# babbu3682/MTD-GAN

Hardware: AMD Instinct MI355X
Metric: GAN train-step imgs/sec (G+D fwd+bwd) @ 64x64 patch (higher is better)
Workload: dtype f32; 1 GPU; Full G+D+PCGrad train step (BASELINE configs[2]; configs[3] when N>1); per_gpu_batch=32, global_batch=32, patch=1x64x64, parallelism=dp1

## Files before the change

mtd-gan_amd/csrc/fft64.h:

```cpp
#pragma once
#include "common.h"

namespace {

__device__ __constant__ const float COS64[32] = {
    1.f, 0.995184727f, 0.98078528f, 0.956940336f, 0.923879533f, 0.881921264f, 0.831469612f, 0.773010453f,
    0.707106781f, 0.634393284f, 0.555570233f, 0.471396737f, 0.382683432f, 0.290284677f, 0.195090322f, 0.0980171403f,
    0.f, -0.0980171403f, -0.195090322f, -0.290284677f, -0.382683432f, -0.471396737f, -0.555570233f, -0.634393284f,
    -0.707106781f, -0.773010453f, -0.831469612f, -0.881921264f, -0.923879533f, -0.956940336f, -0.98078528f, -0.995184727f};
__device__ __constant__ const float SIN64[32] = {
    0.f, 0.0980171403f, 0.195090322f, 0.290284677f, 0.382683432f, 0.471396737f, 0.555570233f, 0.634393284f,
    0.707106781f, 0.773010453f, 0.831469612f, 0.881921264f, 0.923879533f, 0.956940336f, 0.98078528f, 0.995184727f,
    1.f, 0.995184727f, 0.98078528f, 0.956940336f, 0.923879533f, 0.881921264f, 0.831469612f, 0.773010453f,
    0.707106781f, 0.634393284f, 0.555570233f, 0.471396737f, 0.382683432f, 0.290284677f, 0.195090322f, 0.0980171403f};

__host__ __device__ constexpr int brev6(int k) {
    return ((k & 1) << 5) | ((k & 2) << 3) | ((k & 4) << 1) | ((k & 8) >> 1) | ((k & 16) >> 3) | ((k & 32) >> 5);
}

template <int SIGN>
__device__ __forceinline__ void fft64(float (&re)[64], float (&im)[64]) {
#pragma unroll
    for (int s = 0; s < 6; ++s) {
        const int half = 32 >> s;
        const int tstep = 1 << s;
#pragma unroll
        for (int blk = 0; blk < 64; blk += 2 * half) {
#pragma unroll
            for (int j = 0; j < half; ++j) {
                const int i0 = blk + j, i1 = i0 + half;
                const float ar = re[i0], ai = im[i0], br = re[i1], bi = im[i1];
                re[i0] = ar + br;
                im[i0] = ai + bi;
                const float dr = ar - br, di = ai - bi;
                const int tw = j * tstep;
                if (tw == 0) {
                    re[i1] = dr;
                    im[i1] = di;
                } else if (tw == 16) {
                    if (SIGN < 0) { re[i1] = di; im[i1] = -dr; }
                    else { re[i1] = -di; im[i1] = dr; }
                } else {
                    const float c = COS64[tw];
                    const float sn = (SIGN < 0) ? -SIN64[tw] : SIN64[tw];
                    re[i1] = dr * c - di * sn;
                    im[i1] = dr * sn + di * c;
                }
            }
        }
    }
}

__host__ __device__ constexpr int brev4(int k) { return ((k & 1) << 3) | ((k & 2) << 1) | ((k & 4) >> 1) | ((k & 8) >> 3); }

template <int SIGN>
__device__ __forceinline__ void fft16(float (&re)[16], float (&im)[16]) {
#pragma unroll
    for (int s = 0; s < 4; ++s) {
        const int half = 8 >> s;
        const int tstep = 1 << s;
#pragma unroll
        for (int blk = 0; blk < 16; blk += 2 * half) {
#pragma unroll
            for (int j = 0; j < half; ++j) {
                const int i0 = blk + j, i1 = i0 + half;
                const float ar = re[i0], ai = im[i0], br = re[i1], bi = im[i1];
                re[i0] = ar + br;
                im[i0] = ai + bi;
                const float dr = ar - br, di = ai - bi;
                const int tw = j * tstep;
                if (tw == 0) {
                    re[i1] = dr;
                    im[i1] = di;
                } else if (tw == 4) {
                    if (SIGN < 0) { re[i1] = di; im[i1] = -dr; }
                    else { re[i1] = -di; im[i1] = dr; }
                } else {
                    const float c = COS64[4 * tw];
                    const float sn = (SIGN < 0) ? -SIN64[4 * tw] : SIN64[4 * tw];
                    re[i1] = dr * c - di * sn;
                    im[i1] = dr * sn + di * c;
                }
            }
        }
    }
}

__device__ __forceinline__ float quad_bcast(float v, int k) {
    const int x = __builtin_bit_cast(int, v);
    int r;
    switch (k) {
        case 0: r = __builtin_amdgcn_update_dpp(0, x, 0x00, 0xf, 0xf, true); break;
        case 1: r = __builtin_amdgcn_update_dpp(0, x, 0x55, 0xf, 0xf, true); break;
        case 2: r = __builtin_amdgcn_update_dpp(0, x, 0xAA, 0xf, 0xf, true); break;
        default: r = __builtin_amdgcn_update_dpp(0, x, 0xFF, 0xf, 0xf, true); break;
    }
    return __builtin_bit_cast(float, r);
}

template <int SIGN>
__device__ __forceinline__ void fft64_quad(float (&re)[16], float (&im)[16], const float (&tc)[16], const float (&ts)[16], int j) {
    fft16<SIGN>(re, im);
    float gr[16], gi[16];
#pragma unroll
    for (int r = 0; r < 16; ++r) {
        const float fr = re[brev4(r)], fi = im[brev4(r)];
        if (SIGN < 0) { gr[r] = fr * tc[r] + fi * ts[r]; gi[r] = fi * tc[r] - fr * ts[r]; }
        else { gr[r] = fr * tc[r] - fi * ts[r]; gi[r] = fi * tc[r] + fr * ts[r]; }
    }
    const bool odd = (j & 1) != 0;
    const float sgn = (j & 2) ? -1.f : 1.f;
#pragma unroll
    for (int r = 0; r < 16; ++r) {
        const float g0r = quad_bcast(gr[r], 0), g1r = quad_bcast(gr[r], 1), g2r = quad_bcast(gr[r], 2), g3r = quad_bcast(gr[r], 3);
        const float g0i = quad_bcast(gi[r], 0), g1i = quad_bcast(gi[r], 1), g2i = quad_bcast(gi[r], 2), g3i = quad_bcast(gi[r], 3);
        const float ar = g0r + g2r, ai = g0i + g2i, br = g0r - g2r, bi = g0i - g2i;
        const float cr = g1r + g3r, ci = g1i + g3i, dr = g1r - g3r, di = g1i - g3i;
        const float base_r = odd ? br : ar, base_i = odd ? bi : ai;
        const float add_r = odd ? (SIGN < 0 ? di : -di) : cr;
        const float add_i = odd ? (SIGN < 0 ? -dr : dr) : ci;
        re[r] = fmaf(sgn, add_r, base_r);
        im[r] = fmaf(sgn, add_i, base_i);
    }
}

__device__ __forceinline__ void quad_twiddles(int j, float (&tc)[16], float (&ts)[16]) {
#pragma unroll
    for (int r = 0; r < 16; ++r) {
        const int idx = j * r;
        const float s = (idx & 32) ? -1.f : 1.f;
        tc[r] = s * COS64[idx & 31];
        ts[r] = s * SIN64[idx & 31];
    }
}

__device__ __forceinline__ void quad_twiddles_sel(int j, float (&tc)[16], float (&ts)[16]) {
#pragma unroll
    for (int r = 0; r < 16; ++r) {
        const float c1 = COS64[r], s1 = SIN64[r];
        const float c2 = ((2 * r) & 32) ? -COS64[(2 * r) & 31] : COS64[(2 * r) & 31];
        const float s2 = ((2 * r) & 32) ? -SIN64[(2 * r) & 31] : SIN64[(2 * r) & 31];
        const float c3 = ((3 * r) & 32) ? -COS64[(3 * r) & 31] : COS64[(3 * r) & 31];
        const float s3 = ((3 * r) & 32) ? -SIN64[(3 * r) & 31] : SIN64[(3 * r) & 31];
        tc[r] = j == 0 ? 1.f : (j == 1 ? c1 : (j == 2 ? c2 : c3));
        ts[r] = j == 0 ? 0.f : (j == 1 ? s1 : (j == 2 ? s2 : s3));
    }
}

constexpr int NKW = 33;

__device__ __forceinline__ void rfft_rows_body(const float* __restrict__ x, int x_ld, float* __restrict__ R, int npairs, int col_weight,
                                               int pair, int c) {
    if (pair >= npairs) return;
    const int b = pair >> 5, h = (pair & 31) * 2;
    float re[64], im[64];
    const float* r0 = x + ((long long)(b * 64 + h) * 64) * x_ld + c;
    const float* r1 = r0 + (long long)64 * x_ld;
#pragma unroll
    for (int w = 0; w < 64; ++w) {
        re[w] = r0[(long long)w * x_ld];
        im[w] = r1[(long long)w * x_ld];
    }
    fft64<-1>(re, im);
    float* o0 = R + ((long long)(b * NKW) * 64 + h) * 64 + c;
#pragma unroll
    for (int kw = 0; kw <= 32; ++kw) {
        const int km = (64 - kw) & 63;
        const float zkr = re[brev6(kw)], zki = im[brev6(kw)];
        const float zmr = re[brev6(km)], zmi = im[brev6(km)];
        float sc = 0.125f * 0.5f;
        if (col_weight && kw != 0 && kw != 32) sc *= 2.f;
        const float ar = (zkr + zmr) * sc, ai = (zki - zmi) * sc;
        const float br = (zki + zmi) * sc, bi = (zmr - zkr) * sc;
        float* o = o0 + (long long)kw * 64 * 64;
        o[0] = ar;
        o[32] = ai;
        o[64] = br;
        o[64 + 32] = bi;
    }
}

}
```

mtd-gan_amd/csrc/resfft4.hip:

```cpp
#include "common.h"
#include "fft64.h"

namespace {

constexpr int XLD4 = 65;
constexpr int MIX_SLAB4 = 64 * 64 + 128;
typedef __attribute__((address_space(3))) float lds_float4k;

__device__ __forceinline__ void dma_columns(const float* gsrc, float* lds_dst, int wave, int lane, bool two) {
    const int n = two ? 32 : 16;
    for (int i = wave; i < n; i += 4)
        __builtin_amdgcn_global_load_lds(gsrc + i * 256 + lane * 4, (lds_float4k*)(lds_dst + i * 256), 16, 0, 0);
}

__device__ __forceinline__ void store_rows32(const float* lds_rows, int ld, float* gdst, int lane) {
#pragma unroll
    for (int it = 0; it < 8; ++it) {
        const int row = it * 4 + (lane >> 4), q = lane & 15;
        const float* s = lds_rows + row * ld + 4 * q;
        const f32x4 v = {s[0], s[1], s[2], s[3]};
        *reinterpret_cast<f32x4*>(gdst + row * 64 + 4 * q) = v;
    }
}

__device__ __forceinline__ void stagger_wait(int lin, int d, int m) {
    if (d > 0) {
        const int n = ((lin >> 8) % m) * d;
        for (int i = 0; i < n; ++i) __builtin_amdgcn_s_sleep(16);
    }
}

__device__ __forceinline__ int mask_word(int k2, int kh, int o) {
    const int i = kh >> 5, r32 = kh & 31;
    const int e = (r32 & 3) + 4 * (r32 >> 3);
    return ((k2 * 2 + i) * 2 + (o >> 5)) * 16 + e;
}
__device__ __forceinline__ int mask_bit(int kh, int o) { return (o & 31) + 32 * (((kh & 31) >> 2) & 1); }

template <int COLS>
__global__ __launch_bounds__(128 * COLS, 3) void spec_mix_fwd4_kernel(const float* __restrict__ R, const float* __restrict__ w2t,
                                                               const float* __restrict__ b2, float* __restrict__ T,
                                                               float* __restrict__ S_save, unsigned long long* __restrict__ zmask,
                                                               int stg_d, int stg_m) {
    __shared__ __attribute__((aligned(1024))) float Xs[COLS * 64 * XLD4];
    float* const Xin = Xs;
    const int tid = threadIdx.x, lane = tid & 63;
    const int wave = __builtin_amdgcn_readfirstlane(tid >> 6);
    const int b = blockIdx.y;
    const int kw0 = COLS == 2 ? 2 * (int)blockIdx.x : (int)blockIdx.x;
    const int unit = b * 17 + (kw0 >> 1);
    const int kpos = COLS == 2 ? 0 : (kw0 & 1);
    const bool two = COLS == 2 && (kw0 + 1) < NKW;
    const long long cb0 = ((long long)(b * NKW + kw0) * 64) * 64;
    {
        const int n = two ? 32 : 16;
        for (int i = wave; i < n; i += 2 * COLS)
            __builtin_amdgcn_global_load_lds(R + cb0 + i * 256 + lane * 4, (lds_float4k*)(Xin + i * 256), 16, 0, 0);
    }
    stagger_wait(blockIdx.y * gridDim.x + blockIdx.x, stg_d, stg_m);
    const int f = tid >> 2, j = tid & 3, kwl = f >> 5, c = f & 31;
    const bool valid = kwl == 0 || two;
    float tc[16], ts[16];
    quad_twiddles(j, tc, ts);
    const int l31 = lane & 31, kh2 = lane >> 5;
    const int k2 = wave >> 1, ih = wave & 1;
    const bool mix_valid = k2 == 0 || two;
    asm volatile("s_waitcnt vmcnt(0)" ::: "memory");
    __syncthreads();
    float re[16], im[16];
    {
        const float* src = Xin + kwl * 4096 + j * 64 + c;
#pragma unroll
        for (int m = 0; m < 16; ++m) {
            re[m] = valid ? src[m * 256] : 0.f;
            im[m] = valid ? src[m * 256 + 32] : 0.f;
        }
        __syncthreads();
        fft64_quad<-1>(re, im, tc, ts, j);
#pragma unroll
        for (int r = 0; r < 16; ++r) {
            const int kh = 16 * j + r;
            const float sr = re[r] * 0.125f, si = im[r] * 0.125f;
            Xs[(kwl * 64 + kh) * XLD4 + c] = sr;
            Xs[(kwl * 64 + kh) * XLD4 + 32 + c] = si;
        }
    }
    float wf0[32], wf1[32];
#pragma unroll
    for (int kk = 0; kk < 32; ++kk) {
        wf0[kk] = w2t[(2 * kk + kh2) * 64 + l31];
        wf1[kk] = w2t[(2 * kk + kh2) * 64 + 32 + l31];
    }
    __syncthreads();
    if (mix_valid) {
        if (S_save) store_rows32(Xs + (k2 * 64 + ih * 32) * XLD4, XLD4, S_save + cb0 + (k2 * 64 + ih * 32) * 64, lane);
        f32x16 acc[2];
#pragma unroll
        for (int jj = 0; jj < 2; ++jj)
#pragma unroll
            for (int e = 0; e < 16; ++e) acc[jj][e] = 0.f;
        const float* arow = Xs + (k2 * 64 + ih * 32 + l31) * XLD4 + kh2;
#pragma unroll
        for (int kk = 0; kk < 32; ++kk) {
            const float a0 = arow[2 * kk];
            acc[0] = mfma32(a0, wf0[kk], acc[0]);
            acc[1] = mfma32(a0, wf1[kk], acc[1]);
        }
        __builtin_amdgcn_wave_barrier();
#pragma unroll
        for (int jj = 0; jj < 2; ++jj) {
            const int o = jj * 32 + l31;
            const float bo = b2[o];
#pragma unroll
            for (int e = 0; e < 16; ++e) {
                const int kh = ih * 32 + mfma32_row(e, lane);
                const float z = acc[jj][e] + bo;
                if (zmask) {
                    const unsigned long long bm = __ballot(z > 0.f);
                    if (lane == 0) zmask[(long long)unit * 128 + (((k2 + kpos) * 2 + ih) * 2 + jj) * 16 + e] = bm;
                }
                Xs[(k2 * 64 + kh) * XLD4 + o] = z > 0.f ? z : 0.f;
            }
        }
    }
    __syncthreads();
    {
        const float* src = Xs + (kwl * 64 + j) * XLD4 + c;
#pragma unroll
        for (int m = 0; m < 16; ++m) {
            re[m] = src[4 * m * XLD4];
            im[m] = src[4 * m * XLD4 + 32];
        }
        __syncthreads();
        fft64_quad<+1>(re, im, tc, ts, j);
        float* st = Xin + kwl * 4096 + c;
#pragma unroll
        for (int r = 0; r < 16; ++r) {
            const int h = 16 * j + r;
            st[h * 64] = re[r] * 0.125f;
            st[h * 64 + 32] = im[r] * 0.125f;
        }
    }
    __syncthreads();
    if (mix_valid) store_rows32(Xin + (k2 * 64 + ih * 32) * 64, 64, T + cb0 + (k2 * 64 + ih * 32) * 64, lane);
}

__global__ __launch_bounds__(256, 3) void spec_mix_bwd4_kernel(const float* __restrict__ gR, const float* __restrict__ w2,
                                                               const float* __restrict__ S_save,
                                                               const unsigned long long* __restrict__ zmask, float* __restrict__ gT,
                                                               float* __restrict__ ws, int stg_d, int stg_m) {
    __shared__ __attribute__((aligned(1024))) float Gs[2 * 64 * XLD4];
    __shared__ unsigned long long Zm[128];
    float* const Xin = Gs;
    const int tid = threadIdx.x, lane = tid & 63;
    const int wave = __builtin_amdgcn_readfirstlane(tid >> 6);
    const int b = blockIdx.y, unit = b * gridDim.x + blockIdx.x;
    const bool two = (2 * blockIdx.x + 1) < NKW;
    const long long cb0 = ((long long)(b * NKW + 2 * blockIdx.x) * 64) * 64;
    float* slab = ws + (long long)unit * MIX_SLAB4;
    dma_columns(gR + cb0, Xin, wave, lane, two);
    if (tid < 128) Zm[tid] = zmask[(long long)unit * 128 + tid];
    stagger_wait(unit, stg_d, stg_m);
    const int f = tid >> 2, j = tid & 3, kwl = f >> 5, c = f & 31;
    const bool valid = kwl == 0 || two;
    const int l31 = lane & 31, kh2 = lane >> 5;
    asm volatile("s_waitcnt vmcnt(0)" ::: "memory");
    __syncthreads();
    float re[16], im[16];
    const int io = wave >> 1, jk = wave & 1;
    float sf[32];
    {
        const float* sp = S_save + cb0 + kh2 * 64 + jk * 32 + l31;
#pragma unroll
        for (int kk = 0; kk < 32; ++kk) sf[kk] = sp[2 * kk * 64];
    }
    __builtin_amdgcn_sched_barrier(0);
    {
        float tc[16], ts[16];
        quad_twiddles(j, tc, ts);
        const float* src = Xin + kwl * 4096 + j * 64 + c;
#pragma unroll
        for (int m = 0; m < 16; ++m) {
            re[m] = valid ? src[m * 256] : 0.f;
            im[m] = valid ? src[m * 256 + 32] : 0.f;
        }
        __syncthreads();
        fft64_quad<-1>(re, im, tc, ts, j);
        float dbr = 0.f, dbi = 0.f;
#pragma unroll
        for (int r = 0; r < 16; ++r) {
            const int kh = 16 * j + r;
            float gr = re[r] * 0.125f, gi = im[r] * 0.125f;
            const unsigned long long mr = Zm[mask_word(kwl, kh, c)], mi = Zm[mask_word(kwl, kh, 32 + c)];
            const int bit = mask_bit(kh, c);
            gr = (valid && ((mr >> bit) & 1ull)) ? gr : 0.f;
            gi = (valid && ((mi >> bit) & 1ull)) ? gi : 0.f;
            dbr += gr;
            dbi += gi;
            Gs[(kwl * 64 + kh) * XLD4 + c] = gr;
            Gs[(kwl * 64 + kh) * XLD4 + 32 + c] = gi;
        }
        const float sr = ((quad_bcast(dbr, 0) + quad_bcast(dbr, 1)) + quad_bcast(dbr, 2)) + quad_bcast(dbr, 3);
        const float si = ((quad_bcast(dbi, 0) + quad_bcast(dbi, 1)) + quad_bcast(dbi, 2)) + quad_bcast(dbi, 3);
        if (j == 0) {
            slab[64 * 64 + kwl * 64 + c] = sr;
            slab[64 * 64 + kwl * 64 + 32 + c] = si;
        }
    }
    const int k2 = wave >> 1, ih = wave & 1;
    const bool mix_valid = k2 == 0 || two;
    f32x16 accd[2];
#pragma unroll
    for (int jj = 0; jj < 2; ++jj)
#pragma unroll
        for (int e = 0; e < 16; ++e) accd[jj][e] = 0.f;
    {
        float wf0[32], wf1[32];
#pragma unroll
        for (int kk = 0; kk < 32; ++kk) {
            wf0[kk] = w2[(2 * kk + kh2) * 64 + l31];
            wf1[kk] = w2[(2 * kk + kh2) * 64 + 32 + l31];
        }
        __syncthreads();
        if (mix_valid) {
            const float* arow = Gs + (k2 * 64 + ih * 32 + l31) * XLD4 + kh2;
#pragma unroll
            for (int kk = 0; kk < 32; ++kk) {
                const float a0 = arow[2 * kk];
                accd[0] = mfma32(a0, wf0[kk], accd[0]);
                accd[1] = mfma32(a0, wf1[kk], accd[1]);
            }
        }
    }
    {
        f32x16 accw;
#pragma unroll
        for (int e = 0; e < 16; ++e) accw[e] = 0.f;
        float sg[32];
        if (two) {
            const float* sp = S_save + cb0 + 4096 + kh2 * 64 + jk * 32 + l31;
#pragma unroll
            for (int kk = 0; kk < 32; ++kk) sg[kk] = sp[2 * kk * 64];
        }
        {
            const float* ga = Gs + kh2 * XLD4 + io * 32 + l31;
#pragma unroll
            for (int kk = 0; kk < 32; ++kk) accw = mfma32(ga[2 * kk * XLD4], sf[kk], accw);
        }
        if (two) {
            const float* ga = Gs + (64 + kh2) * XLD4 + io * 32 + l31;
#pragma unroll
            for (int kk = 0; kk < 32; ++kk) accw = mfma32(ga[2 * kk * XLD4], sg[kk], accw);
        }
#pragma unroll
        for (int e = 0; e < 16; ++e) slab[(io * 32 + mfma32_row(e, lane)) * 64 + jk * 32 + l31] = accw[e];
    }
    __syncthreads();
    if (mix_valid) {
#pragma unroll
        for (int jj = 0; jj < 2; ++jj)
#pragma unroll
            for (int e = 0; e < 16; ++e) Gs[(k2 * 64 + ih * 32 + mfma32_row(e, lane)) * XLD4 + jj * 32 + l31] = accd[jj][e];
    }
    __syncthreads();
    {
        float tc[16], ts[16];
        quad_twiddles(j, tc, ts);
        const float* src = Gs + (kwl * 64 + j) * XLD4 + c;
#pragma unroll
        for (int m = 0; m < 16; ++m) {
            re[m] = src[4 * m * XLD4];
            im[m] = src[4 * m * XLD4 + 32];
        }
        __syncthreads();
        fft64_quad<+1>(re, im, tc, ts, j);
        const int kw = 2 * blockIdx.x + kwl;
        const float sc = (kw == 0 || kw == 32) ? 0.125f : 0.0625f;
        float* st = Xin + kwl * 4096 + c;
#pragma unroll
        for (int r = 0; r < 16; ++r) {
            const int h = 16 * j + r;
            st[h * 64] = re[r] * sc;
            st[h * 64 + 32] = im[r] * sc;
        }
    }
    __syncthreads();
    if (mix_valid) store_rows32(Xin + (k2 * 64 + ih * 32) * 64, 64, gT + cb0 + (k2 * 64 + ih * 32) * 64, lane);
}

}

extern "C" size_t mtd_spec_mix_zmask_bytes(int B) { return B > 0 ? (size_t)B * 17 * 128 * sizeof(unsigned long long) : 0; }

extern "C" int mtd_spec_mix_fwd4(const float* R, const float* w2t, const float* b2, float* T, float* S_save, void* zmask, int B,
                                 void* stream) {
    if (!R || !w2t || !b2 || !T || B <= 0) return MTD_EINVAL;
    if (!aligned16(R)) return MTD_EALIGN;
    static const int env_cols = [] { const char* e = mtd_lab_env("MTD_SPECMIX_COLS"); return e ? atoi(e) : 1; }();
    static const int stg_d = [] { const char* e = mtd_lab_env("MTD_SPECMIX_STAGGER"); return e ? atoi(e) : 0; }();
    static const int stg_m = [] { const char* e = mtd_lab_env("MTD_SPECMIX_STAGGER_MOD"); return e ? atoi(e) : 2; }();
    if (env_cols == 2)
        hipLaunchKernelGGL((spec_mix_fwd4_kernel<2>), dim3(17, B), dim3(256), 0, (hipStream_t)stream, R, w2t, b2, T, S_save,
                           (unsigned long long*)zmask, stg_d, stg_m);
    else
        hipLaunchKernelGGL((spec_mix_fwd4_kernel<1>), dim3(NKW, B), dim3(128), 0, (hipStream_t)stream, R, w2t, b2, T, S_save,
                           (unsigned long long*)zmask, stg_d, stg_m);
    MTD_LAUNCH_CHECK();
    return MTD_OK;
}

extern "C" int mtd_spec_mix_bwd4(const float* gR, const float* w2, const float* S_save, const void* zmask, float* gT, float* ws, int B,
                                 void* stream) {
    if (!gR || !w2 || !S_save || !zmask || !gT || !ws || B <= 0) return MTD_EINVAL;
    if (!aligned16(gR) || !aligned16(S_save)) return MTD_EALIGN;
    static const int stg_d = [] { const char* e = mtd_lab_env("MTD_SPECMIX_STAGGER_BWD"); return e ? atoi(e) : 0; }();
    static const int stg_m = [] { const char* e = mtd_lab_env("MTD_SPECMIX_STAGGER_MOD"); return e ? atoi(e) : 2; }();
    hipLaunchKernelGGL(spec_mix_bwd4_kernel, dim3(17, B), dim3(256), 0, (hipStream_t)stream, gR, w2, S_save,
                       (const unsigned long long*)zmask, gT, ws, stg_d, stg_m);
    MTD_LAUNCH_CHECK();
    return MTD_OK;
}
```

Before: 1243 img/s.

## Pack real spectral columns, fold FFT scaling into twiddles, use DPP FMA butterflies

```diff
diff --git a/mtd-gan_amd/csrc/fft64.h b/mtd-gan_amd/csrc/fft64.h
--- a/mtd-gan_amd/csrc/fft64.h
+++ b/mtd-gan_amd/csrc/fft64.h
@@ -3,12 +3,12 @@
 
 namespace {
 
-__device__ __constant__ const float COS64[32] = {
+__device__ __constant__ constexpr float COS64[32] = {
     1.f, 0.995184727f, 0.98078528f, 0.956940336f, 0.923879533f, 0.881921264f, 0.831469612f, 0.773010453f,
     0.707106781f, 0.634393284f, 0.555570233f, 0.471396737f, 0.382683432f, 0.290284677f, 0.195090322f, 0.0980171403f,
     0.f, -0.0980171403f, -0.195090322f, -0.290284677f, -0.382683432f, -0.471396737f, -0.555570233f, -0.634393284f,
     -0.707106781f, -0.773010453f, -0.831469612f, -0.881921264f, -0.923879533f, -0.956940336f, -0.98078528f, -0.995184727f};
-__device__ __constant__ const float SIN64[32] = {
+__device__ __constant__ constexpr float SIN64[32] = {
     0.f, 0.0980171403f, 0.195090322f, 0.290284677f, 0.382683432f, 0.471396737f, 0.555570233f, 0.634393284f,
     0.707106781f, 0.773010453f, 0.831469612f, 0.881921264f, 0.923879533f, 0.956940336f, 0.98078528f, 0.995184727f,
     1.f, 0.995184727f, 0.98078528f, 0.956940336f, 0.923879533f, 0.881921264f, 0.831469612f, 0.773010453f,
@@ -98,8 +98,50 @@
     return __builtin_bit_cast(float, r);
 }
 
-template <int SIGN>
-__device__ __forceinline__ void fft64_quad(float (&re)[16], float (&im)[16], const float (&tc)[16], const float (&ts)[16], int j) {
+template <int CTRL>
+__device__ __forceinline__ float quad_perm(float v) {
+    return __builtin_bit_cast(float, __builtin_amdgcn_update_dpp(0, __builtin_bit_cast(int, v), CTRL, 0xf, 0xf, true));
+}
+
+struct QuadTw { float v[4][32]; };
+constexpr QuadTw make_quad_tw() {
+    QuadTw t{};
+    for (int j = 0; j < 4; ++j)
+        for (int r = 0; r < 16; ++r) {
+            const int idx = j * r;
+            const float s = (((idx & 32) != 0) != (j >= 2)) ? -0.125f : 0.125f;
+            t.v[j][r] = s * COS64[idx & 31];
+            t.v[j][16 + r] = s * SIN64[idx & 31];
+        }
+    return t;
+}
+__device__ __constant__ const QuadTw QTW8 = make_quad_tw();
+
+__device__ __forceinline__ void quad_twiddles8(int j, float (&tc)[16], float (&ts)[16]) {
+    const f32x4* q = reinterpret_cast<const f32x4*>(QTW8.v[j]);
+#pragma unroll
+    for (int i = 0; i < 4; ++i) {
+        const f32x4 c = q[i], s = q[4 + i];
+#pragma unroll
+        for (int e = 0; e < 4; ++e) { tc[4 * i + e] = c[e]; ts[4 * i + e] = s[e]; }
+    }
+}
+
+struct QuadCoef { float c1, ca, cb, cbn; };
+template <int SIGN>
+__device__ __forceinline__ QuadCoef quad_coef(int j) {
+    QuadCoef q;
+    q.c1 = (j & 2) ? 1.f : -1.f;
+    q.ca = (j & 1) ? 0.f : ((j & 2) ? -1.f : 1.f);
+    const float sb = (j & 2) ? -1.f : 1.f;
+    q.cb = (j & 1) ? (SIGN < 0 ? sb : -sb) : 0.f;
+    q.cbn = -q.cb;
+    return q;
+}
+
+#define MTD_QDPP "row_mask:0xf bank_mask:0xf bound_ctrl:1\n\t"
+template <int SIGN>
+__device__ __forceinline__ void fft64_quad(float (&re)[16], float (&im)[16], const float (&tc)[16], const float (&ts)[16], const QuadCoef qc) {
     fft16<SIGN>(re, im);
     float gr[16], gi[16];
 #pragma unroll
@@ -108,44 +150,48 @@
         if (SIGN < 0) { gr[r] = fr * tc[r] + fi * ts[r]; gi[r] = fi * tc[r] - fr * ts[r]; }
         else { gr[r] = fr * tc[r] - fi * ts[r]; gi[r] = fi * tc[r] + fr * ts[r]; }
     }
-    const bool odd = (j & 1) != 0;
-    const float sgn = (j & 2) ? -1.f : 1.f;
-#pragma unroll
-    for (int r = 0; r < 16; ++r) {
-        const float g0r = quad_bcast(gr[r], 0), g1r = quad_bcast(gr[r], 1), g2r = quad_bcast(gr[r], 2), g3r = quad_bcast(gr[r], 3);
-        const float g0i = quad_bcast(gi[r], 0), g1i = quad_bcast(gi[r], 1), g2i = quad_bcast(gi[r], 2), g3i = quad_bcast(gi[r], 3);
-        const float ar = g0r + g2r, ai = g0i + g2i, br = g0r - g2r, bi = g0i - g2i;
-        const float cr = g1r + g3r, ci = g1i + g3i, dr = g1r - g3r, di = g1i - g3i;
-        const float base_r = odd ? br : ar, base_i = odd ? bi : ai;
-        const float add_r = odd ? (SIGN < 0 ? di : -di) : cr;
-        const float add_i = odd ? (SIGN < 0 ? -dr : dr) : ci;
-        re[r] = fmaf(sgn, add_r, base_r);
-        im[r] = fmaf(sgn, add_i, base_i);
-    }
-}
-
-__device__ __forceinline__ void quad_twiddles(int j, float (&tc)[16], float (&ts)[16]) {
-#pragma unroll
-    for (int r = 0; r < 16; ++r) {
-        const int idx = j * r;
-        const float s = (idx & 32) ? -1.f : 1.f;
-        tc[r] = s * COS64[idx & 31];
-        ts[r] = s * SIN64[idx & 31];
-    }
-}
-
-__device__ __forceinline__ void quad_twiddles_sel(int j, float (&tc)[16], float (&ts)[16]) {
-#pragma unroll
-    for (int r = 0; r < 16; ++r) {
-        const float c1 = COS64[r], s1 = SIN64[r];
-        const float c2 = ((2 * r) & 32) ? -COS64[(2 * r) & 31] : COS64[(2 * r) & 31];
-        const float s2 = ((2 * r) & 32) ? -SIN64[(2 * r) & 31] : SIN64[(2 * r) & 31];
-        const float c3 = ((3 * r) & 32) ? -COS64[(3 * r) & 31] : COS64[(3 * r) & 31];
-        const float s3 = ((3 * r) & 32) ? -SIN64[(3 * r) & 31] : SIN64[(3 * r) & 31];
-        tc[r] = j == 0 ? 1.f : (j == 1 ? c1 : (j == 2 ? c2 : c3));
-        ts[r] = j == 0 ? 0.f : (j == 1 ? s1 : (j == 2 ? s2 : s3));
-    }
-}
+#pragma unroll
+    for (int r = 0; r < 16; r += 4) {
+        asm volatile(
+            "s_nop 4\n\t"
+            "v_fmac_f32_dpp %0, %0, %16 quad_perm:[2,3,0,1] " MTD_QDPP
+            "v_fmac_f32_dpp %1, %1, %16 quad_perm:[2,3,0,1] " MTD_QDPP
+            "v_fmac_f32_dpp %2, %2, %16 quad_perm:[2,3,0,1] " MTD_QDPP
+            "v_fmac_f32_dpp %3, %3, %16 quad_perm:[2,3,0,1] " MTD_QDPP
+            "v_fmac_f32_dpp %4, %4, %16 quad_perm:[2,3,0,1] " MTD_QDPP
+            "v_fmac_f32_dpp %5, %5, %16 quad_perm:[2,3,0,1] " MTD_QDPP
+            "v_fmac_f32_dpp %6, %6, %16 quad_perm:[2,3,0,1] " MTD_QDPP
+            "v_fmac_f32_dpp %7, %7, %16 quad_perm:[2,3,0,1] " MTD_QDPP
+            "v_mov_b32_dpp %8, %0 quad_perm:[0,2,0,2] " MTD_QDPP
+            "v_mov_b32_dpp %9, %1 quad_perm:[0,2,0,2] " MTD_QDPP
+            "v_mov_b32_dpp %10, %2 quad_perm:[0,2,0,2] " MTD_QDPP
+            "v_mov_b32_dpp %11, %3 quad_perm:[0,2,0,2] " MTD_QDPP
+            "v_mov_b32_dpp %12, %4 quad_perm:[0,2,0,2] " MTD_QDPP
+            "v_mov_b32_dpp %13, %5 quad_perm:[0,2,0,2] " MTD_QDPP
+            "v_mov_b32_dpp %14, %6 quad_perm:[0,2,0,2] " MTD_QDPP
+            "v_mov_b32_dpp %15, %7 quad_perm:[0,2,0,2] " MTD_QDPP
+            "v_fmac_f32_dpp %8, %0, %17 quad_perm:[1,3,1,3] " MTD_QDPP
+            "v_fmac_f32_dpp %9, %1, %17 quad_perm:[1,3,1,3] " MTD_QDPP
+            "v_fmac_f32_dpp %10, %2, %17 quad_perm:[1,3,1,3] " MTD_QDPP
+            "v_fmac_f32_dpp %11, %3, %17 quad_perm:[1,3,1,3] " MTD_QDPP
+            "v_fmac_f32_dpp %12, %4, %17 quad_perm:[1,3,1,3] " MTD_QDPP
+            "v_fmac_f32_dpp %13, %5, %17 quad_perm:[1,3,1,3] " MTD_QDPP
+            "v_fmac_f32_dpp %14, %6, %17 quad_perm:[1,3,1,3] " MTD_QDPP
+            "v_fmac_f32_dpp %15, %7, %17 quad_perm:[1,3,1,3] " MTD_QDPP
+            "v_fmac_f32_dpp %8, %1, %18 quad_perm:[1,3,1,3] " MTD_QDPP
+            "v_fmac_f32_dpp %9, %0, %19 quad_perm:[1,3,1,3] " MTD_QDPP
+            "v_fmac_f32_dpp %10, %3, %18 quad_perm:[1,3,1,3] " MTD_QDPP
+            "v_fmac_f32_dpp %11, %2, %19 quad_perm:[1,3,1,3] " MTD_QDPP
+            "v_fmac_f32_dpp %12, %5, %18 quad_perm:[1,3,1,3] " MTD_QDPP
+            "v_fmac_f32_dpp %13, %4, %19 quad_perm:[1,3,1,3] " MTD_QDPP
+            "v_fmac_f32_dpp %14, %7, %18 quad_perm:[1,3,1,3] " MTD_QDPP
+            "v_fmac_f32_dpp %15, %6, %19 quad_perm:[1,3,1,3] row_mask:0xf bank_mask:0xf bound_ctrl:1"
+            : "+v"(gr[r]), "+v"(gi[r]), "+v"(gr[r + 1]), "+v"(gi[r + 1]), "+v"(gr[r + 2]), "+v"(gi[r + 2]), "+v"(gr[r + 3]), "+v"(gi[r + 3]),
+              "=&v"(re[r]), "=&v"(im[r]), "=&v"(re[r + 1]), "=&v"(im[r + 1]), "=&v"(re[r + 2]), "=&v"(im[r + 2]), "=&v"(re[r + 3]), "=&v"(im[r + 3])
+            : "v"(qc.c1), "v"(qc.ca), "v"(qc.cb), "v"(qc.cbn));
+    }
+}
+#undef MTD_QDPP
 
 constexpr int NKW = 33;
 
diff --git a/mtd-gan_amd/csrc/resfft4.hip b/mtd-gan_amd/csrc/resfft4.hip
--- a/mtd-gan_amd/csrc/resfft4.hip
+++ b/mtd-gan_amd/csrc/resfft4.hip
@@ -1,5 +1,6 @@
 #include "common.h"
 #include "fft64.h"
+#include <type_traits>
 
 namespace {
 
@@ -37,22 +38,47 @@
 }
 __device__ __forceinline__ int mask_bit(int kh, int o) { return (o & 31) + 32 * (((kh & 31) >> 2) & 1); }
 
-template <int COLS>
-__global__ __launch_bounds__(128 * COLS, 3) void spec_mix_fwd4_kernel(const float* __restrict__ R, const float* __restrict__ w2t,
+template <int W>
+__device__ __forceinline__ void put_lane(int& m, unsigned v) {
+    asm volatile("v_writelane_b32 %0, %1, %2" : "+v"(m) : "s"(v), "n"(W));
+}
+template <int W>
+__device__ __forceinline__ void put_lane_now(int& m, unsigned v) {
+    asm volatile("s_nop 7\n\tv_writelane_b32 %0, %1, %2" : "+v"(m) : "s"(v), "n"(W));
+}
+template <int I, int N, typename F>
+__device__ __forceinline__ void static_for(F&& f) {
+    if constexpr (I < N) {
+        f(std::integral_constant<int, I>{});
+        static_for<I + 1, N>(f);
+    }
+}
+
+__device__ __forceinline__ void store_mask32(unsigned long long* dst, int lo, int hi, int lane) {
+    if (lane < 32) dst[lane] = ((unsigned long long)(unsigned)hi << 32) | (unsigned)lo;
+}
+
+template <int COLS, bool PACK>
+__global__ __launch_bounds__(128 * COLS, PACK ? 2 : 3) void spec_mix_fwd4_kernel(const float* __restrict__ R, const float* __restrict__ w2t,
                                                                const float* __restrict__ b2, float* __restrict__ T,
                                                                float* __restrict__ S_save, unsigned long long* __restrict__ zmask,
                                                                int stg_d, int stg_m) {
-    __shared__ __attribute__((aligned(1024))) float Xs[COLS * 64 * XLD4];
+    extern __shared__ __attribute__((aligned(1024))) float Xs[];
     float* const Xin = Xs;
     const int tid = threadIdx.x, lane = tid & 63;
     const int wave = __builtin_amdgcn_readfirstlane(tid >> 6);
     const int b = blockIdx.y;
+    const bool packed = PACK && blockIdx.x == 0;
     const int kw0 = COLS == 2 ? 2 * (int)blockIdx.x : (int)blockIdx.x;
     const int unit = b * 17 + (kw0 >> 1);
     const int kpos = COLS == 2 ? 0 : (kw0 & 1);
     const bool two = COLS == 2 && (kw0 + 1) < NKW;
     const long long cb0 = ((long long)(b * NKW + kw0) * 64) * 64;
-    {
+    if (packed) {
+        const float* src = R + cb0 + (lane >> 4) * 64 + ((lane & 8) ? 32 * 4096 : 0) + 4 * (lane & 7);
+        for (int i = wave; i < 16; i += 2)
+            __builtin_amdgcn_global_load_lds(src + i * 256, (lds_float4k*)(Xin + i * 256), 16, 0, 0);
+    } else {
         const int n = two ? 32 : 16;
         for (int i = wave; i < n; i += 2 * COLS)
             __builtin_amdgcn_global_load_lds(R + cb0 + i * 256 + lane * 4, (lds_float4k*)(Xin + i * 256), 16, 0, 0);
@@ -61,7 +87,12 @@
     const int f = tid >> 2, j = tid & 3, kwl = f >> 5, c = f & 31;
     const bool valid = kwl == 0 || two;
     float tc[16], ts[16];
-    quad_twiddles(j, tc, ts);
+    quad_twiddles8(j, tc, ts);
+    if (packed) {
+#pragma unroll
+        for (int r = 0; r < 16; ++r) { tc[r] *= 0.5f; ts[r] *= 0.5f; }
+    }
+    const QuadCoef qf = quad_coef<-1>(j), qi = quad_coef<+1>(j);
     const int l31 = lane & 31, kh2 = lane >> 5;
     const int k2 = wave >> 1, ih = wave & 1;
     const bool mix_valid = k2 == 0 || two;
@@ -76,13 +107,26 @@
             im[m] = valid ? src[m * 256 + 32] : 0.f;
         }
         __syncthreads();
-        fft64_quad<-1>(re, im, tc, ts, j);
-#pragma unroll
-        for (int r = 0; r < 16; ++r) {
-            const int kh = 16 * j + r;
-            const float sr = re[r] * 0.125f, si = im[r] * 0.125f;
-            Xs[(kwl * 64 + kh) * XLD4 + c] = sr;
-            Xs[(kwl * 64 + kh) * XLD4 + 32 + c] = si;
+        fft64_quad<-1>(re, im, tc, ts, qf);
+        if (packed) {
+#pragma unroll
+            for (int r = 0; r < 16; ++r) {
+                const int kh = 16 * j + r;
+                const float zr = re[r], zi = im[r];
+                const float mr = r ? quad_perm<0x1B>(re[16 - r]) : quad_perm<0x6C>(re[0]);
+                const float mi = r ? quad_perm<0x1B>(im[16 - r]) : quad_perm<0x6C>(im[0]);
+                Xs[kh * XLD4 + c] = zr + mr;
+                Xs[kh * XLD4 + 32 + c] = zi - mi;
+                Xs[(64 + kh) * XLD4 + c] = zi + mi;
+                Xs[(64 + kh) * XLD4 + 32 + c] = mr - zr;
+            }
+        } else {
+#pragma unroll
+            for (int r = 0; r < 16; ++r) {
+                const int kh = 16 * j + r;
+                Xs[(kwl * 64 + kh) * XLD4 + c] = re[r];
+                Xs[(kwl * 64 + kh) * XLD4 + 32 + c] = im[r];
+            }
         }
     }
     float wf0[32], wf1[32];
@@ -92,7 +136,93 @@
         wf1[kk] = w2t[(2 * kk + kh2) * 64 + 32 + l31];
     }
     __syncthreads();
-    if (mix_valid) {
+    if (packed) {
+        const long long cbp = ((long long)(b * NKW + 32 * ih) * 64) * 64;
+        if (S_save) {
+            store_rows32(Xs + ih * 64 * XLD4, XLD4, S_save + cbp, lane);
+            store_rows32(Xs + (ih * 64 + 32) * XLD4, XLD4, S_save + cbp + 32 * 64, lane);
+        }
+        f32x16 accp[2], accq[2];
+#pragma unroll
+        for (int jj = 0; jj < 2; ++jj)
+#pragma unroll
+            for (int e = 0; e < 16; ++e) accp[jj][e] = accq[jj][e] = 0.f;
+        const float* arow = Xs + (ih * 64 + l31) * XLD4 + kh2;
+#pragma unroll
+        for (int kk = 0; kk < 16; ++kk) {
+            const float a0 = arow[2 * kk], a1 = arow[32 + 2 * kk];
+            accp[0] = mfma32(a0, wf0[kk], accp[0]);
+            accp[1] = mfma32(a0, wf1[kk], accp[1]);
+            accq[0] = mfma32(a1, wf0[16 + kk], accq[0]);
+            accq[1] = mfma32(a1, wf1[16 + kk], accq[1]);
+        }
+        float e0 = 0.f, e1 = 0.f;
+        {
+            const float* x32 = Xs + (ih * 64 + 32) * XLD4 + kh2;
+#pragma unroll
+            for (int kk = 0; kk < 16; ++kk) {
+                const float xv = x32[2 * kk];
+                e0 = fmaf(wf0[kk], xv, e0);
+                e1 = fmaf(wf1[kk], xv, e1);
+            }
+            const float o0 = __shfl_xor(e0, 32), o1 = __shfl_xor(e1, 32);
+            e0 = kh2 ? o0 + e0 : e0 + o0;
+            e1 = kh2 ? o1 + e1 : e1 + o1;
+        }
+        __builtin_amdgcn_wave_barrier();
+        int ma_lo = 0, ma_hi = 0, mb_lo = 0, mb_hi = 0;
+        static_for<0, 2>([&](auto jj_) {
+            constexpr int jj = decltype(jj_)::value;
+            const int o = jj * 32 + l31;
+            const float bo = b2[o];
+            const float z32 = (jj ? e1 : e0) + bo;
+            const unsigned long long bm32 = __ballot(z32 > 0.f);
+            if (zmask) put_lane_now<jj * 16>(mb_lo, (unsigned)bm32);
+            if (jj == 0) {
+                Xs[(ih * 64 + 32) * XLD4 + lane] = kh2 ? 0.f : 2.f * fmaxf(z32, 0.f);
+            }
+            static_for<0, 4>([&](auto g_) {
+                constexpr int g = decltype(g_)::value;
+                float z1[4], z2[4];
+                unsigned long long bm1[4], bm2[4];
+#pragma unroll
+                for (int a = 0; a < 4; ++a) {
+                    z1[a] = (accp[jj][4 * g + a] + accq[jj][4 * g + a]) + bo;
+                    z2[a] = (accp[jj][4 * g + a] - accq[jj][4 * g + a]) + bo;
+                    bm1[a] = __ballot(z1[a] > 0.f);
+                    bm2[a] = __ballot(z2[a] > 0.f);
+                }
+                if (zmask) {
+                    __builtin_amdgcn_sched_barrier(0);
+                    static_for<0, 4>([&](auto a_) {
+                        constexpr int a = decltype(a_)::value, e = 4 * g + a;
+                        put_lane<jj * 16 + e>(ma_lo, (unsigned)bm1[a]);
+                        put_lane<jj * 16 + e>(ma_hi, (unsigned)(bm1[a] >> 32));
+                        if constexpr (a != 0) {
+                            constexpr int w = jj * 16 + (4 - a) + 4 * (3 - g);
+                            put_lane<w>(mb_lo, (unsigned)(bm2[a] >> 32));
+                            put_lane<w>(mb_hi, (unsigned)bm2[a]);
+                        } else {
+                            put_lane<jj * 16 + 4 * (3 - g)>(mb_hi, (unsigned)(bm2[a] >> 32));
+                            if constexpr (g != 0) put_lane<jj * 16 + 4 * (4 - g)>(mb_lo, (unsigned)bm2[a]);
+                        }
+                    });
+                    __builtin_amdgcn_sched_barrier(0);
+                }
+#pragma unroll
+                for (int a = 0; a < 4; ++a) {
+                    const int kh = mfma32_row(4 * g + a, lane);
+                    const float y1 = fmaxf(z1[a], 0.f), y2 = fmaxf(z2[a], 0.f);
+                    Xs[(ih * 64 + kh) * XLD4 + o] = jj ? y1 - y2 : y1 + y2;
+                }
+            });
+        });
+        if (zmask) {
+            unsigned long long* zm = zmask + (long long)(b * 17 + 16 * ih) * 128;
+            store_mask32(zm, ma_lo, ma_hi, lane);
+            store_mask32(zm + 32, mb_lo, mb_hi, lane);
+        }
+    } else if (mix_valid) {
         if (S_save) store_rows32(Xs + (k2 * 64 + ih * 32) * XLD4, XLD4, S_save + cb0 + (k2 * 64 + ih * 32) * 64, lane);
         f32x16 acc[2];
 #pragma unroll
@@ -107,42 +237,83 @@
             acc[1] = mfma32(a0, wf1[kk], acc[1]);
         }
         __builtin_amdgcn_wave_barrier();
-#pragma unroll
-        for (int jj = 0; jj < 2; ++jj) {
+        int m_lo = 0, m_hi = 0;
+        static_for<0, 2>([&](auto jj_) {
+            constexpr int jj = decltype(jj_)::value;
             const int o = jj * 32 + l31;
             const float bo = b2[o];
-#pragma unroll
-            for (int e = 0; e < 16; ++e) {
-                const int kh = ih * 32 + mfma32_row(e, lane);
-                const float z = acc[jj][e] + bo;
+            static_for<0, 2>([&](auto g_) {
+                constexpr int g = decltype(g_)::value;
+                float z[8];
+                unsigned long long bm[8];
+#pragma unroll
+                for (int u = 0; u < 8; ++u) {
+                    z[u] = acc[jj][8 * g + u] + bo;
+                    bm[u] = __ballot(z[u] > 0.f);
+                }
                 if (zmask) {
-                    const unsigned long long bm = __ballot(z > 0.f);
-                    if (lane == 0) zmask[(long long)unit * 128 + (((k2 + kpos) * 2 + ih) * 2 + jj) * 16 + e] = bm;
+                    __builtin_amdgcn_sched_barrier(0);
+                    static_for<0, 8>([&](auto u_) {
+                        constexpr int u = decltype(u_)::value;
+                        put_lane<jj * 16 + 8 * g + u>(m_lo, (unsigned)bm[u]);
+                        put_lane<jj * 16 + 8 * g + u>(m_hi, (unsigned)(bm[u] >> 32));
+                    });
+                    __builtin_amdgcn_sched_barrier(0);
                 }
-                Xs[(k2 * 64 + kh) * XLD4 + o] = z > 0.f ? z : 0.f;
-            }
-        }
-    }
-    __syncthreads();
-    {
-        const float* src = Xs + (kwl * 64 + j) * XLD4 + c;
-#pragma unroll
-        for (int m = 0; m < 16; ++m) {
-            re[m] = src[4 * m * XLD4];
-            im[m] = src[4 * m * XLD4 + 32];
+#pragma unroll
+                for (int u = 0; u < 8; ++u) {
+                    const int kh = ih * 32 + mfma32_row(8 * g + u, lane);
+                    Xs[(k2 * 64 + kh) * XLD4 + o] = z[u] > 0.f ? z[u] : 0.f;
+                }
+            });
+        });
+        if (zmask) store_mask32(zmask + (long long)unit * 128 + ((k2 + kpos) * 2 + ih) * 32, m_lo, m_hi, lane);
+    }
+    __syncthreads();
+    {
+        if (packed) {
+#pragma unroll
+            for (int m = 0; m < 16; ++m) {
+                const int k = 4 * m + j;
+                const bool low = m < 8 || (m == 8 && j == 0);
+                const float* u = Xs + (low ? k : 64 - k) * XLD4 + c;
+                const float* v = u + 64 * XLD4;
+                const float sg = low ? 1.f : -1.f;
+                re[m] = fmaf(-sg, v[32], u[0]);
+                im[m] = fmaf(sg, u[32], v[0]);
+            }
+        } else {
+            const float* src = Xs + (kwl * 64 + j) * XLD4 + c;
+#pragma unroll
+            for (int m = 0; m < 16; ++m) {
+                re[m] = src[4 * m * XLD4];
+                im[m] = src[4 * m * XLD4 + 32];
+            }
         }
         __syncthreads();
-        fft64_quad<+1>(re, im, tc, ts, j);
+        fft64_quad<+1>(re, im, tc, ts, qi);
+        const int kw = kw0 + kwl;
+        const bool keep_im = packed || (kw != 0 && kw != 32);
         float* st = Xin + kwl * 4096 + c;
 #pragma unroll
         for (int r = 0; r < 16; ++r) {
             const int h = 16 * j + r;
-            st[h * 64] = re[r] * 0.125f;
-            st[h * 64 + 32] = im[r] * 0.125f;
-        }
-    }
-    __syncthreads();
-    if (mix_valid) store_rows32(Xin + (k2 * 64 + ih * 32) * 64, 64, T + cb0 + (k2 * 64 + ih * 32) * 64, lane);
+            st[h * 64] = re[r];
+            st[h * 64 + 32] = keep_im ? im[r] : 0.f;
+        }
+    }
+    __syncthreads();
+    if (packed) {
+#pragma unroll
+        for (int it = 0; it < 16; ++it) {
+            const int row = ih * 32 + (it & 7) * 4 + (lane >> 4), q = lane & 15, col = it >> 3;
+            const float* s = Xin + row * 64 + col * 32 + 4 * (q & 7);
+            const f32x4 v = q < 8 ? f32x4{s[0], s[1], s[2], s[3]} : f32x4{0.f, 0.f, 0.f, 0.f};
+            *reinterpret_cast<f32x4*>(T + cb0 + (long long)col * 32 * 4096 + row * 64 + 4 * q) = v;
+        }
+    } else if (mix_valid) {
+        store_rows32(Xin + (k2 * 64 + ih * 32) * 64, 64, T + cb0 + (k2 * 64 + ih * 32) * 64, lane);
+    }
 }
 
 __global__ __launch_bounds__(256, 3) void spec_mix_bwd4_kernel(const float* __restrict__ gR, const float* __restrict__ w2,
@@ -175,9 +346,10 @@
         for (int kk = 0; kk < 32; ++kk) sf[kk] = sp[2 * kk * 64];
     }
     __builtin_amdgcn_sched_barrier(0);
-    {
-        float tc[16], ts[16];
-        quad_twiddles(j, tc, ts);
+    float tc[16], ts[16];
+    quad_twiddles8(j, tc, ts);
+    const QuadCoef qf = quad_coef<-1>(j), qi = quad_coef<+1>(j);
+    {
         const float* src = Xin + kwl * 4096 + j * 64 + c;
 #pragma unroll
         for (int m = 0; m < 16; ++m) {
@@ -185,12 +357,12 @@
             im[m] = valid ? src[m * 256 + 32] : 0.f;
         }
         __syncthreads();
-        fft64_quad<-1>(re, im, tc, ts, j);
+        fft64_quad<-1>(re, im, tc, ts, qf);
         float dbr = 0.f, dbi = 0.f;
 #pragma unroll
         for (int r = 0; r < 16; ++r) {
             const int kh = 16 * j + r;
-            float gr = re[r] * 0.125f, gi = im[r] * 0.125f;
+            float gr = re[r], gi = im[r];
             const unsigned long long mr = Zm[mask_word(kwl, kh, c)], mi = Zm[mask_word(kwl, kh, 32 + c)];
             const int bit = mask_bit(kh, c);
             gr = (valid && ((mr >> bit) & 1ull)) ? gr : 0.f;
@@ -264,8 +436,6 @@
     }
     __syncthreads();
     {
-        float tc[16], ts[16];
-        quad_twiddles(j, tc, ts);
         const float* src = Gs + (kwl * 64 + j) * XLD4 + c;
 #pragma unroll
         for (int m = 0; m < 16; ++m) {
@@ -273,15 +443,17 @@
             im[m] = src[4 * m * XLD4 + 32];
         }
         __syncthreads();
-        fft64_quad<+1>(re, im, tc, ts, j);
+        fft64_quad<+1>(re, im, tc, ts, qi);
         const int kw = 2 * blockIdx.x + kwl;
-        const float sc = (kw == 0 || kw == 32) ? 0.125f : 0.0625f;
+        const bool real_col = kw == 0 || kw == 32;
+        const float sc = real_col ? 1.f : 0.5f;
+        const float sci = real_col ? 0.f : 0.5f;
         float* st = Xin + kwl * 4096 + c;
 #pragma unroll
         for (int r = 0; r < 16; ++r) {
             const int h = 16 * j + r;
             st[h * 64] = re[r] * sc;
-            st[h * 64 + 32] = im[r] * sc;
+            st[h * 64 + 32] = im[r] * sci;
         }
     }
     __syncthreads();
@@ -291,20 +463,36 @@
 }
 
 extern "C" size_t mtd_spec_mix_zmask_bytes(int B) { return B > 0 ? (size_t)B * 17 * 128 * sizeof(unsigned long long) : 0; }
+
+static int spec_mix_lds_bytes(int need, int units) {
+    constexpr int LDS_CU = 160 * 1024;
+    const int cap = (units + 255) / 256;
+    const int req = (LDS_CU / (cap + 1) / 1024 + 1) * 1024;
+    return (req >= need && (long long)req * cap <= LDS_CU) ? req : need;
+}
 
 extern "C" int mtd_spec_mix_fwd4(const float* R, const float* w2t, const float* b2, float* T, float* S_save, void* zmask, int B,
                                  void* stream) {
     if (!R || !w2t || !b2 || !T || B <= 0) return MTD_EINVAL;
     if (!aligned16(R)) return MTD_EALIGN;
     static const int env_cols = [] { const char* e = mtd_lab_env("MTD_SPECMIX_COLS"); return e ? atoi(e) : 1; }();
+    static const int env_pack = [] { const char* e = mtd_lab_env("MTD_SPECMIX_PACK"); return e ? atoi(e) : 0; }();
     static const int stg_d = [] { const char* e = mtd_lab_env("MTD_SPECMIX_STAGGER"); return e ? atoi(e) : 0; }();
     static const int stg_m = [] { const char* e = mtd_lab_env("MTD_SPECMIX_STAGGER_MOD"); return e ? atoi(e) : 2; }();
-    if (env_cols == 2)
-        hipLaunchKernelGGL((spec_mix_fwd4_kernel<2>), dim3(17, B), dim3(256), 0, (hipStream_t)stream, R, w2t, b2, T, S_save,
+    constexpr int IMG = 64 * XLD4 * (int)sizeof(float);
+    if (env_cols == 2) {
+        hipLaunchKernelGGL((spec_mix_fwd4_kernel<2, false>), dim3(17, B), dim3(256), 2 * IMG, (hipStream_t)stream, R, w2t, b2, T, S_save,
                            (unsigned long long*)zmask, stg_d, stg_m);
-    else
-        hipLaunchKernelGGL((spec_mix_fwd4_kernel<1>), dim3(NKW, B), dim3(128), 0, (hipStream_t)stream, R, w2t, b2, T, S_save,
+    } else if (env_pack && 32 * B <= 1024) {
+        static const hipError_t attr = hipFuncSetAttribute(reinterpret_cast<const void*>(&spec_mix_fwd4_kernel<1, true>),
+                                                           hipFuncAttributeMaxDynamicSharedMemorySize, 160 * 1024);
+        if (attr != hipSuccess) return (int)attr;
+        hipLaunchKernelGGL((spec_mix_fwd4_kernel<1, true>), dim3(32, B), dim3(128), spec_mix_lds_bytes(2 * IMG, 32 * B), (hipStream_t)stream,
+                           R, w2t, b2, T, S_save, (unsigned long long*)zmask, stg_d, stg_m);
+    } else {
+        hipLaunchKernelGGL((spec_mix_fwd4_kernel<1, false>), dim3(NKW, B), dim3(128), IMG, (hipStream_t)stream, R, w2t, b2, T, S_save,
                            (unsigned long long*)zmask, stg_d, stg_m);
+    }
     MTD_LAUNCH_CHECK();
     return MTD_OK;
 }
```

Result: no change. 1246 img/s (median of 6 runs) (+0.2%).
